# thobotics/geometry_rl

Measured on NVIDIA B200. Metric: fwd+bwd+TRPL update samples/sec (policy fwd+bwd, TRPL projection, losses, critic, Adam), higher is better.
Workload: dtype bf16

## Files before the change

### geometry_rl_b200/csrc/grl_conv_node_tc.cu

```cuda
#include <cuda.h>

#include "grl_common.cuh"
#include "grl_tc.cuh"

namespace grl {

constexpr int kLDX = 72;

constexpr int kNF2Threads = 512;
constexpr int kK1 = 80;

struct NodeFwd2Group {
  union {
    struct {
      float X1[kTM * kC];
      float X2[kTM * kLDX];
    } x;
    __half A1[kTM * kK1];
  } u;
};

struct NodeFwd2Smem {
  __half W1h[kH * kK1];
  __half W2h[kC * kH];
  NodeFwd2Group g[2];
  float b2[kC], bias[kC], lng[kC], lnb[kC];
  uint64_t bar[2][2];
  uint64_t bar_x[2];
  uint64_t bar_d[2];
  uint32_t tmem_base;
};

__device__ __forceinline__ void stage_x1_dense(float* __restrict__ X1, const float* __restrict__ src, int cnt, int gt,
                                               uint64_t* bar) {
  if (gt == 0) {
    tc::mbar_expect_tx(bar, (uint32_t)cnt * kRow * 4u);
    tc::bulk_g2s(X1, src, (uint32_t)cnt * kRow * 4u, bar);
  }
  if (cnt < kTE) {
#pragma unroll
    for (int i = 0; i < 8; ++i) {
      const int f = gt + 256 * i;
      if ((f >> 8) >= cnt) *reinterpret_cast<float4*>(X1 + 4 * f) = make_float4(0.f, 0.f, 0.f, 0.f);
    }
  }
}

template <bool kAcc>
__global__ void __launch_bounds__(kNF2Threads, 1) fbconv_node_fwd_tc2_kernel(const GrlConvDesc d, const __grid_constant__ CUtensorMap tm_xd) {
  extern __shared__ unsigned char smem_raw[];
  NodeFwd2Smem& s = *reinterpret_cast<NodeFwd2Smem*>(
      smem_raw + ((1024u - (tc::smem_u32(smem_raw) & 1023u)) & 1023u));
  const int tid = threadIdx.x;
  const int grp = tid >> 8, gt = tid & 255, gw = gt >> 5, lane = tid & 31;
  NodeFwd2Group& G = s.g[grp];
  const int bar_id = 1 + grp;

  if (tid == 0) {
    tc::mbar_init(&s.bar[0][0], 1);
    tc::mbar_init(&s.bar[0][1], 1);
    tc::mbar_init(&s.bar[1][0], 1);
    tc::mbar_init(&s.bar[1][1], 1);
    tc::mbar_init(&s.bar_x[0], 1);
    tc::mbar_init(&s.bar_x[1], 1);
    tc::mbar_init(&s.bar_d[0], 1);
    tc::mbar_init(&s.bar_d[1], 1);
    tc::fence_mbar_init();
  }
  if (tid < 32) tc::tmem_alloc(&s.tmem_base, 512);
  tc::stage_weight_f16(s.W1h, d.w1, kH, kC, kC);
  tc::stage_weight_f16(s.W2h, d.w2, kC, kH, kH);
  for (int n = tid; n < kH; n += kNF2Threads) {
    const float b = d.b1[n];
    const __half hi = __float2half_rn(b);
    const __half lo = __float2half_rn(b - __half2float(hi));
    const __half z = __float2half_rn(0.f);
    const __half2 h[4] = {__halves2half2(hi, lo), __halves2half2(z, z), __halves2half2(z, z), __halves2half2(z, z)};
    *reinterpret_cast<uint4*>(s.W1h + ((size_t)8 * kH + n) * 8) = tc::pack_h8(h);
    *reinterpret_cast<uint4*>(s.W1h + ((size_t)9 * kH + n) * 8) = make_uint4(0u, 0u, 0u, 0u);
  }
  if (tid < kC) { s.b2[tid] = d.b2[tid]; s.bias[tid] = d.bias[tid]; s.lng[tid] = d.ln_g[tid]; s.lnb[tid] = d.ln_b[tid]; }
  const int fc = gt & 63, pq = gt >> 6;
  unsigned long long fk2[kO][2];
#pragma unroll
  for (int o = 0; o < kO; ++o)
#pragma unroll
    for (int pi = 0; pi < 2; ++pi)
      fk2[o][pi] = pack2(__ldg(d.fiber_kernel + ((size_t)(o * kO + 4 * pq + 2 * pi)) * kC + fc) * 0.0625f,
                         __ldg(d.fiber_kernel + ((size_t)(o * kO + 4 * pq + 2 * pi + 1)) * kC + fc) * 0.0625f);

  const int n_tiles = (d.n_dst + kTE - 1) / kTE;
  const int tile_stride = 2 * gridDim.x;
  int tile = 2 * blockIdx.x + grp;
  tc::fence_async_smem();
  tc::tc_fence_before();
  __syncthreads();
  tc::tc_fence_after();
  if (tile < n_tiles)
    stage_x1_dense(G.u.x.X1, d.x1 + (size_t)tile * kTE * kRow, min(kTE, d.n_dst - tile * kTE), gt, &s.bar_x[grp]);
  const uint32_t tmem = s.tmem_base + 256u * grp;
  const uint32_t a1_addr = tc::smem_u32(G.u.A1);
  const uint32_t w1_addr = tc::smem_u32(s.W1h), w2_addr = tc::smem_u32(s.W2h);
  const int q = gw & 3, hh = gw >> 2;
  const int row = 32 * q + lane;
  const uint32_t lane_addr = tmem + ((uint32_t)(32 * q) << 16);
  uint32_t parity = 0;

  for (; tile < n_tiles; tile += tile_stride) {
    const int n0 = tile * kTE;
    if (gt == 0) {
      tc::prefetch_l2(d.x_dst + (size_t)n0 * kRow, (uint32_t)min(kTE, d.n_dst - n0) * kRow * 4u);
      const int nt = tile + tile_stride;
      if (nt < n_tiles) tc::prefetch_l2(d.x1 + (size_t)nt * kTE * kRow, (uint32_t)min(kTE, d.n_dst - nt * kTE) * kRow * 4u);
    }
    tc::mbar_wait(&s.bar_x[grp], parity);
    tc::group_sync(bar_id, 256);

    {
      const float bias_c = s.bias[fc];
#pragma unroll 2
      for (int j = 0; j < kTE; ++j) {
        unsigned long long a01 = pack2(0.f, 0.f), a23 = a01;
#pragma unroll
        for (int o = 0; o < kO; ++o) {
          const float x = G.u.x.X1[(16 * j + o) * kC + fc];
          const unsigned long long xx = pack2(x, x);
          a01 = ffma2(xx, fk2[o][0], a01);
          a23 = ffma2(xx, fk2[o][1], a23);
        }
        float a0, a1, a2, a3;
        unpack2(a01, a0, a1);
        unpack2(a23, a2, a3);
        float* o2 = G.u.x.X2 + (16 * j + 4 * pq) * kLDX + fc;
        o2[0 * kLDX] = a0 + bias_c;
        o2[1 * kLDX] = a1 + bias_c;
        o2[2 * kLDX] = a2 + bias_c;
        o2[3 * kLDX] = a3 + bias_c;
      }
    }
    tc::group_sync(bar_id, 256);

    {
      const int r = gt >> 1, h = gt & 1;
      float4 v[8];
      float sum = 0.f;
#pragma unroll
      for (int i = 0; i < 8; ++i) {
        v[i] = ld4(G.u.x.X2 + r * kLDX + 4 * (2 * i + h));
        sum += (v[i].x + v[i].y) + (v[i].z + v[i].w);
      }
      if (d.x2 && n0 + (r >> 4) < d.n_dst) {
        float* xo = d.x2 + (size_t)(n0 + (r >> 4)) * kRow + (r & 15) * kC + 4 * h;
#pragma unroll
        for (int i = 0; i < 8; ++i) st4(xo + 8 * i, v[i]);
      }
      sum += __shfl_xor_sync(0xffffffffu, sum, 1);
      const float mean = sum * (1.0f / 64.0f);
      float sq = 0.f;
#pragma unroll
      for (int i = 0; i < 8; ++i) {
        v[i].x -= mean; v[i].y -= mean; v[i].z -= mean; v[i].w -= mean;
        sq += (v[i].x * v[i].x + v[i].y * v[i].y) + (v[i].z * v[i].z + v[i].w * v[i].w);
      }
      sq += __shfl_xor_sync(0xffffffffu, sq, 1);
      const float rstd = rsqrtf(sq * (1.0f / 64.0f) + 1e-5f);
#pragma unroll
      for (int i = 0; i < 8; ++i) {
        const int c = 4 * (2 * i + h);
        const float4 g = ld4(s.lng + c), b = ld4(s.lnb + c);
        const __half2 p0 = __floats2half2_rn(v[i].x * rstd * g.x + b.x, v[i].y * rstd * g.y + b.y);
        const __half2 p1 = __floats2half2_rn(v[i].z * rstd * g.z + b.z, v[i].w * rstd * g.w + b.w);
        uint2 pk;
        pk.x = *reinterpret_cast<const uint32_t*>(&p0);
        pk.y = *reinterpret_cast<const uint32_t*>(&p1);
        *reinterpret_cast<uint2*>(G.u.A1 + ((size_t)i * kTM + r) * 8 + 4 * h) = pk;
      }
      *reinterpret_cast<uint4*>(G.u.A1 + ((size_t)(8 + h) * kTM + r) * 8) = make_uint4(h == 0 ? 0x3C003C00u : 0u, 0u, 0u, 0u);
    }
    tc::fence_async_smem();
    tc::tc_fence_before();
    tc::group_sync(bar_id, 256);
    if (gt == 0) {
      tc::tc_fence_after();
      tc::issue_mma_rolled(tmem, tc::view_k(a1_addr, kTM), tc::view_k(w1_addr, kH), tc::idesc_f16_ex(128, kH, 0, 0, 0, 0), kK1 / 16, false);
      tc::mma_commit(&s.bar[grp][0]);
      tc::mbar_expect_tx(&s.bar_d[grp], 2u * kTM * 32u * 4u);
      tc::tma_load_2d(G.u.x.X2, &tm_xd, 0, n0 * kO, &s.bar_d[grp]);
      tc::tma_load_2d(G.u.x.X2 + kTM * 32, &tm_xd, 32, n0 * kO, &s.bar_d[grp]);
    }
    tc::mbar_wait(&s.bar[grp][0], parity);
    tc::tc_fence_after();
    {
      const int nt = tile + tile_stride;
      if (nt < n_tiles) {
        tc::fence_async_smem();
        stage_x1_dense(G.u.x.X1, d.x1 + (size_t)nt * kTE * kRow, min(kTE, d.n_dst - nt * kTE), gt, &s.bar_x[grp]);
      }
    }
    {
#pragma unroll 2
      for (int i = 0; i < 8; ++i) {
        const int c0 = 128 * hh + 16 * i;
        float v[16];
        tc::tmem_ld16(lane_addr + c0, v);
        uint32_t r[8];
#pragma unroll
        for (int e = 0; e < 4; ++e) {
          const __half2 a = tc::gelu_h2(__floats2half2_rn(v[2 * e], v[2 * e + 1]));
          const __half2 b = tc::gelu_h2(__floats2half2_rn(v[8 + 2 * e], v[8 + 2 * e + 1]));
          r[e] = *reinterpret_cast<const uint32_t*>(&a);
          r[4 + e] = *reinterpret_cast<const uint32_t*>(&b);
        }
        tc::tmem_st8(lane_addr + 128 * hh + 8 * i, r);
      }
      tc::tmem_st_wait();
    }
    tc::tc_fence_before();
    tc::group_sync(bar_id, 256);
    if (gt == 0) {
      tc::tc_fence_after();
      const tc::OpView w2v = tc::view_k(w2_addr, kC);
      tc::OpView w2hi = w2v;
      w2hi.addr += 8 * w2v.adv;
      tc::issue_mma_ts(tmem + 64, tmem, w2v, tc::idesc_f16_ex(128, kC, 0, 0, 0, 0), 8, false);
      tc::issue_mma_ts(tmem + 64, tmem + 128, w2hi, tc::idesc_f16_ex(128, kC, 0, 0, 0, 0), 8, true);
      tc::mma_commit(&s.bar[grp][1]);
    }
    const int node = n0 + (row >> 4);
    const bool live = node < d.n_dst;
    const size_t off = (size_t)(live ? node : 0) * kRow + (row & 15) * kC + 32 * hh;
    tc::mbar_wait(&s.bar[grp][1], parity);
    tc::tc_fence_after();
    tc::mbar_wait(&s.bar_d[grp], parity);
    const float* xrow = G.u.x.X2 + hh * (kTM * 32) + row * 32;
#pragma unroll
    for (int i = 0; i < 2; ++i) {
      float v[16];
      tc::tmem_ld16(lane_addr + 64 + 32 * hh + 16 * i, v);
      if (live) {
#pragma unroll
        for (int e = 0; e < 4; ++e) {
          const float4 bb = ld4(s.b2 + 32 * hh + 16 * i + 4 * e);
          float4 x = ld4(xrow + (((4 * i + e) ^ (row & 7)) << 2));
          if (kAcc) {
            const float4 old = ldg4(d.out + off + 16 * i + 4 * e);
            x.x += old.x; x.y += old.y; x.z += old.z; x.w += old.w;
          }
          st4(d.out + off + 16 * i + 4 * e, make_float4(x.x + (v[4 * e] + bb.x), x.y + (v[4 * e + 1] + bb.y),
                                                       x.z + (v[4 * e + 2] + bb.z), x.w + (v[4 * e + 3] + bb.w)));
        }
      }
    }
    tc::tc_fence_before();
    parity ^= 1u;
  }
  cp_async_wait_all();
  tc::tc_fence_before();
  __syncthreads();
  if (tid < 32) tc::tmem_dealloc(s.tmem_base, 512);
}

}

extern "C" int grl_fbconv_node_fwd_tc(const GrlConvDesc* d, grl_stream_t stream) {
  GRL_REQUIRE(d && d->n_dst > 0, GRL_EINVAL, "grl_fbconv_node_fwd_tc: bad descriptor");
  GRL_REQUIRE(d->x1 && d->fiber_kernel && d->bias && d->ln_g && d->ln_b && d->w1 && d->b1 && d->w2 && d->b2 && d->x_dst &&
                  d->out, GRL_EINVAL, "grl_fbconv_node_fwd_tc: null pointer");
  const int n_tiles = (d->n_dst + grl::kTE - 1) / grl::kTE;
  const int smem2 = (int)sizeof(grl::NodeFwd2Smem) + 1024;
  if (grl::ensure_dynamic_smem((const void*)grl::fbconv_node_fwd_tc2_kernel<false>, smem2) != GRL_OK) return GRL_ECUDA;
  if (grl::ensure_dynamic_smem((const void*)grl::fbconv_node_fwd_tc2_kernel<true>, smem2) != GRL_OK) return GRL_ECUDA;
  alignas(64) CUtensorMap tm_xd;
  if (grl::make_row_tensor_map(&tm_xd, d->x_dst, d->n_dst, grl::kTM) != GRL_OK) return GRL_ECUDA;
  int grid = grl::sm_count();
  if (2 * grid > n_tiles) grid = (n_tiles + 1) / 2;
  if (d->accumulate_out) grl::fbconv_node_fwd_tc2_kernel<true><<<grid, grl::kNF2Threads, smem2, (cudaStream_t)stream>>>(*d, tm_xd);
  else grl::fbconv_node_fwd_tc2_kernel<false><<<grid, grl::kNF2Threads, smem2, (cudaStream_t)stream>>>(*d, tm_xd);
  return grl::check_launch("grl_fbconv_node_fwd_tc");
}
```

### geometry_rl_b200/csrc/grl_tc.cuh

```cuda
#pragma once
#include <cuda_bf16.h>
#include <cuda_fp16.h>
#include <cuda_runtime.h>
#include <stdint.h>

namespace grl {
namespace tc {

__device__ __forceinline__ uint32_t smem_u32(const void* p) { return static_cast<uint32_t>(__cvta_generic_to_shared(p)); }

__device__ __forceinline__ void mbar_init(uint64_t* bar, uint32_t count) {
  asm volatile("mbarrier.init.shared::cta.b64 [%0], %1;" ::"r"(smem_u32(bar)), "r"(count) : "memory");
}
__device__ __forceinline__ void fence_mbar_init() { asm volatile("fence.mbarrier_init.release.cluster;" ::: "memory"); }
__device__ __forceinline__ void mbar_wait(uint64_t* bar, uint32_t parity) {
  const uint32_t addr = smem_u32(bar);
  uint32_t done;
  do {
    asm volatile(
        "{\n\t"
        ".reg .pred p;\n\t"
        "mbarrier.try_wait.parity.shared::cta.b64 p, [%1], %2;\n\t"
        "selp.u32 %0, 1, 0, p;\n\t"
        "}"
        : "=r"(done)
        : "r"(addr), "r"(parity)
        : "memory");
  } while (!done);
}

__device__ __forceinline__ void mbar_expect_tx(uint64_t* bar, uint32_t bytes) {
  asm volatile("mbarrier.arrive.expect_tx.shared::cta.b64 _, [%0], %1;" ::"r"(smem_u32(bar)), "r"(bytes) : "memory");
}
__device__ __forceinline__ void bulk_g2s(void* smem_dst, const void* gsrc, uint32_t bytes, uint64_t* bar) {
  asm volatile("cp.async.bulk.shared::cluster.global.mbarrier::complete_tx::bytes [%0], [%1], %2, [%3];" ::"r"(
                   smem_u32(smem_dst)),
               "l"(gsrc), "r"(bytes), "r"(smem_u32(bar))
               : "memory");
}

__device__ __forceinline__ void tma_load_2d(void* smem_dst, const void* tmap, int c0, int c1, uint64_t* bar) {
  asm volatile("cp.async.bulk.tensor.2d.shared::cluster.global.mbarrier::complete_tx::bytes [%0], [%1, {%2, %3}], [%4];" ::"r"(
                   smem_u32(smem_dst)),
               "l"(tmap), "r"(c0), "r"(c1), "r"(smem_u32(bar))
               : "memory");
}
__device__ __forceinline__ void tma_prefetch_desc(const void* tmap) {
  asm volatile("prefetch.tensormap [%0];" ::"l"(tmap) : "memory");
}

__device__ __forceinline__ void fence_async_smem() { asm volatile("fence.proxy.async.shared::cta;" ::: "memory"); }
__device__ __forceinline__ void tc_fence_before() { asm volatile("tcgen05.fence::before_thread_sync;" ::: "memory"); }
__device__ __forceinline__ void tc_fence_after() { asm volatile("tcgen05.fence::after_thread_sync;" ::: "memory"); }

__device__ __forceinline__ void tmem_alloc(uint32_t* smem_dst, uint32_t ncols) {
  asm volatile("tcgen05.alloc.cta_group::1.sync.aligned.shared::cta.b32 [%0], %1;" ::"r"(smem_u32(smem_dst)), "r"(ncols)
               : "memory");
  asm volatile("tcgen05.relinquish_alloc_permit.cta_group::1.sync.aligned;" ::: "memory");
}
__device__ __forceinline__ void tmem_dealloc(uint32_t taddr, uint32_t ncols) {
  asm volatile("tcgen05.dealloc.cta_group::1.sync.aligned.b32 %0, %1;" ::"r"(taddr), "r"(ncols) : "memory");
}

__device__ __forceinline__ uint64_t smem_desc(uint32_t saddr, uint32_t lbo_bytes, uint32_t sbo_bytes) {
  uint64_t d = 0;
  d |= (uint64_t)((saddr >> 4) & 0x3FFF);
  d |= (uint64_t)((lbo_bytes >> 4) & 0x3FFF) << 16;
  d |= (uint64_t)((sbo_bytes >> 4) & 0x3FFF) << 32;
  d |= (uint64_t)1 << 46;
  return d;
}
__host__ __device__ constexpr uint32_t idesc_bf16(int M, int N) {
  return (1u << 4) | (1u << 7) | (1u << 10) | ((uint32_t)(N >> 3) << 17) | ((uint32_t)(M >> 4) << 24);
}

__host__ __device__ constexpr uint32_t idesc_f16_ex(int M, int N, int a_mn, int b_mn, int a_bf16, int b_bf16) {
  return (1u << 4) | ((uint32_t)a_bf16 << 7) | ((uint32_t)b_bf16 << 10) | ((uint32_t)a_mn << 15) | ((uint32_t)b_mn << 16) |
         ((uint32_t)(N >> 3) << 17) | ((uint32_t)(M >> 4) << 24);
}

__device__ __forceinline__ void mma_bf16(uint32_t tmem_d, uint64_t desc_a, uint64_t desc_b, uint32_t idesc, uint32_t accumulate) {
  asm volatile(
      "{\n\t"
      ".reg .pred p;\n\t"
      "setp.ne.b32 p, %4, 0;\n\t"
      "tcgen05.mma.cta_group::1.kind::f16 [%0], %1, %2, %3, p;\n\t"
      "}" ::"r"(tmem_d),
      "l"(desc_a), "l"(desc_b), "r"(idesc), "r"(accumulate)
      : "memory");
}
__device__ __forceinline__ void mma_commit(uint64_t* bar) {
  asm volatile("tcgen05.commit.cta_group::1.mbarrier::arrive::one.shared::cluster.b64 [%0];" ::"r"(smem_u32(bar)) : "memory");
}

template <int N, int K>
__device__ __forceinline__ void issue_gemm(uint32_t tmem_d, uint32_t a_saddr, int a_rows, uint32_t b_saddr, int b_rows,
                                           bool accumulate_first) {
  constexpr uint32_t idesc = idesc_bf16(128, N);
#pragma unroll
  for (int k = 0; k < K / 16; ++k) {
    const uint64_t da = smem_desc(a_saddr + k * 2 * a_rows * 16, a_rows * 16, 128);
    const uint64_t db = smem_desc(b_saddr + k * 2 * b_rows * 16, b_rows * 16, 128);
    mma_bf16(tmem_d, da, db, idesc, (k > 0 || accumulate_first) ? 1u : 0u);
  }
}

struct OpView {
  uint32_t addr, lbo, sbo, adv;
};
__device__ __forceinline__ OpView view_k(uint32_t addr, int rows) { return OpView{addr, (uint32_t)rows * 16u, 128u, (uint32_t)rows * 32u}; }
__device__ __forceinline__ OpView view_mn(uint32_t addr, int rows) { return OpView{addr, 128u, (uint32_t)rows * 16u, 256u}; }
__host__ __device__ constexpr uint32_t idesc_bf16_ex(int M, int N, int a_mn, int b_mn) {
  return idesc_bf16(M, N) | ((uint32_t)a_mn << 15) | ((uint32_t)b_mn << 16);
}
struct Op {
  uint32_t lo, hi, step;
};
__device__ __forceinline__ uint32_t desc_lo(uint32_t saddr, uint32_t lbo_bytes) {
  return ((saddr >> 4) & 0x3FFFu) | (((lbo_bytes >> 4) & 0x3FFFu) << 16);
}
__device__ __forceinline__ uint32_t desc_hi(uint32_t sbo_bytes) { return ((sbo_bytes >> 4) & 0x3FFFu) | (1u << 14); }
__device__ __forceinline__ Op op_k(uint32_t addr, int rows) { return Op{desc_lo(addr, (uint32_t)rows * 16u), desc_hi(128u), (uint32_t)rows * 2u}; }
__device__ __forceinline__ Op op_mn(uint32_t addr, int rows) { return Op{desc_lo(addr, 128u), desc_hi((uint32_t)rows * 16u), 16u}; }
__device__ __forceinline__ void mma_f16_words(uint32_t tmem_d, uint32_t alo, uint32_t ahi, uint32_t blo, uint32_t bhi, uint32_t idesc,
                                              uint32_t accumulate) {
  asm volatile(
      "{\n\t"
      ".reg .pred p;\n\t"
      ".reg .b64 da, db;\n\t"
      "setp.ne.b32 p, %6, 0;\n\t"
      "mov.b64 da, {%1, %2};\n\t"
      "mov.b64 db, {%3, %4};\n\t"
      "tcgen05.mma.cta_group::1.kind::f16 [%0], da, db, %5, p;\n\t"
      "}" ::"r"(tmem_d),
      "r"(alo), "r"(ahi), "r"(blo), "r"(bhi), "r"(idesc), "r"(accumulate)
      : "memory");
}
template <int KSTEPS>
__device__ __forceinline__ void issue_mma_fast(uint32_t tmem_d, const Op& a, const Op& b, uint32_t idesc, bool accumulate_first) {
  mma_f16_words(tmem_d, a.lo, a.hi, b.lo, b.hi, idesc, accumulate_first ? 1u : 0u);
#pragma unroll
  for (int k = 1; k < KSTEPS; ++k) mma_f16_words(tmem_d, a.lo + k * a.step, a.hi, b.lo + k * b.step, b.hi, idesc, 1u);
}
__device__ __forceinline__ void mma_f16_ts(uint32_t tmem_d, uint32_t tmem_a, uint32_t blo, uint32_t bhi, uint32_t idesc,
                                           uint32_t accumulate) {
  asm volatile(
      "{\n\t"
      ".reg .pred p;\n\t"
      ".reg .b64 db;\n\t"
      "setp.ne.b32 p, %5, 0;\n\t"
      "mov.b64 db, {%2, %3};\n\t"
      "tcgen05.mma.cta_group::1.kind::f16 [%0], [%1], db, %4, p;\n\t"
      "}" ::"r"(tmem_d),
      "r"(tmem_a), "r"(blo), "r"(bhi), "r"(idesc), "r"(accumulate)
      : "memory");
}
__device__ __forceinline__ void issue_mma_ts(uint32_t tmem_d, uint32_t tmem_a, const OpView& b, uint32_t idesc, int ksteps,
                                             bool accumulate_first) {
  const uint32_t blo = desc_lo(b.addr, b.lbo), bhi = desc_hi(b.sbo), bs = b.adv >> 4;
#pragma unroll
  for (int k = 0; k < ksteps; ++k)
    mma_f16_ts(tmem_d, tmem_a + 8u * k, blo + k * bs, bhi, idesc, (k > 0 || accumulate_first) ? 1u : 0u);
}

__device__ __forceinline__ void issue_mma(uint32_t tmem_d, const OpView& a, const OpView& b, uint32_t idesc, int ksteps,
                                          bool accumulate_first) {
  const uint32_t alo = desc_lo(a.addr, a.lbo), ahi = desc_hi(a.sbo), blo = desc_lo(b.addr, b.lbo), bhi = desc_hi(b.sbo);
  const uint32_t as = a.adv >> 4, bs = b.adv >> 4;
#pragma unroll
  for (int k = 0; k < ksteps; ++k)
    mma_f16_words(tmem_d, alo + k * as, ahi, blo + k * bs, bhi, idesc, (k > 0 || accumulate_first) ? 1u : 0u);
}
__device__ __forceinline__ void issue_mma_rolled(uint32_t tmem_d, const OpView& a, const OpView& b, uint32_t idesc, int ksteps,
                                                 bool accumulate_first) {
  uint32_t alo = desc_lo(a.addr, a.lbo), blo = desc_lo(b.addr, b.lbo);
  const uint32_t ahi = desc_hi(a.sbo), bhi = desc_hi(b.sbo), as = a.adv >> 4, bs = b.adv >> 4;
  mma_f16_words(tmem_d, alo, ahi, blo, bhi, idesc, accumulate_first ? 1u : 0u);
#pragma unroll 1
  for (int k = 1; k < ksteps; ++k) {
    alo += as;
    blo += bs;
    mma_f16_words(tmem_d, alo, ahi, blo, bhi, idesc, 1u);
  }
}
__device__ __forceinline__ bool elect_one() {
  uint32_t pred;
  asm volatile(
      "{\n\t"
      ".reg .pred p;\n\t"
      "elect.sync _|p, 0xffffffff;\n\t"
      "selp.u32 %0, 1, 0, p;\n\t"
      "}"
      : "=r"(pred));
  return pred != 0;
}

template <int NV>
__device__ __forceinline__ void warp_colsum(float (&v)[NV], int lane) {
  static_assert(NV % 32 == 0, "NV must be a multiple of 32");
#pragma unroll
  for (int step = 0; step < 5; ++step) {
    const int half = NV >> (step + 1);
    const int bit = 16 >> step;
    const bool upper = (lane & bit) != 0;
#pragma unroll
    for (int i = 0; i < half; ++i) {
      const float keep = upper ? v[i + half] : v[i];
      const float send = upper ? v[i] : v[i + half];
      v[i] = keep + __shfl_xor_sync(0xffffffffu, send, bit);
    }
  }
}

__device__ __forceinline__ void tmem_ld16(uint32_t taddr, float (&v)[16]) {
  uint32_t r[16];
  asm volatile(
      "tcgen05.ld.sync.aligned.32x32b.x16.b32 {%0, %1, %2, %3, %4, %5, %6, %7, %8, %9, %10, %11, %12, %13, %14, %15}, [%16];"
      : "=r"(r[0]), "=r"(r[1]), "=r"(r[2]), "=r"(r[3]), "=r"(r[4]), "=r"(r[5]), "=r"(r[6]), "=r"(r[7]), "=r"(r[8]),
        "=r"(r[9]), "=r"(r[10]), "=r"(r[11]), "=r"(r[12]), "=r"(r[13]), "=r"(r[14]), "=r"(r[15])
      : "r"(taddr)
      : "memory");
  asm volatile("tcgen05.wait::ld.sync.aligned;" ::: "memory");
#pragma unroll
  for (int i = 0; i < 16; ++i) v[i] = __uint_as_float(r[i]);
}

__device__ __forceinline__ void tmem_st16(uint32_t taddr, const uint32_t (&r)[16]) {
  asm volatile(
      "tcgen05.st.sync.aligned.32x32b.x16.b32 [%0], {%1, %2, %3, %4, %5, %6, %7, %8, %9, %10, %11, %12, %13, %14, %15, %16};" ::"r"(taddr),
      "r"(r[0]), "r"(r[1]), "r"(r[2]), "r"(r[3]), "r"(r[4]), "r"(r[5]), "r"(r[6]), "r"(r[7]), "r"(r[8]), "r"(r[9]), "r"(r[10]),
      "r"(r[11]), "r"(r[12]), "r"(r[13]), "r"(r[14]), "r"(r[15])
      : "memory");
}
__device__ __forceinline__ void tmem_st8(uint32_t taddr, const uint32_t (&r)[8]) {
  asm volatile("tcgen05.st.sync.aligned.32x32b.x8.b32 [%0], {%1, %2, %3, %4, %5, %6, %7, %8};" ::"r"(taddr), "r"(r[0]), "r"(r[1]),
               "r"(r[2]), "r"(r[3]), "r"(r[4]), "r"(r[5]), "r"(r[6]), "r"(r[7])
               : "memory");
}
__device__ __forceinline__ void tmem_st_wait() { asm volatile("tcgen05.wait::st.sync.aligned;" ::: "memory"); }
__device__ __forceinline__ void tmem_ld16_raw(uint32_t taddr, uint32_t (&r)[16]) {
  asm volatile(
      "tcgen05.ld.sync.aligned.32x32b.x16.b32 {%0, %1, %2, %3, %4, %5, %6, %7, %8, %9, %10, %11, %12, %13, %14, %15}, [%16];"
      : "=r"(r[0]), "=r"(r[1]), "=r"(r[2]), "=r"(r[3]), "=r"(r[4]), "=r"(r[5]), "=r"(r[6]), "=r"(r[7]), "=r"(r[8]),
        "=r"(r[9]), "=r"(r[10]), "=r"(r[11]), "=r"(r[12]), "=r"(r[13]), "=r"(r[14]), "=r"(r[15])
      : "r"(taddr)
      : "memory");
  asm volatile("tcgen05.wait::ld.sync.aligned;" ::: "memory");
}
__device__ __forceinline__ void mbar_arrive(uint64_t* bar) {
  asm volatile("mbarrier.arrive.shared::cta.b64 _, [%0];" ::"r"(smem_u32(bar)) : "memory");
}

__device__ __forceinline__ void prefetch_l2(const void* gptr, uint32_t bytes) {
  asm volatile("cp.async.bulk.prefetch.L2.global [%0], %1;" ::"l"(gptr), "r"(bytes) : "memory");
}

__device__ __forceinline__ void group_sync(int id, int count) { asm volatile("bar.sync %0, %1;" ::"r"(id), "r"(count) : "memory"); }

__device__ __forceinline__ __half2 tanh_h2(__half2 x) {
  uint32_t r;
  asm("tanh.approx.f16x2 %0, %1;" : "=r"(r) : "r"(*reinterpret_cast<uint32_t*>(&x)));
  return *reinterpret_cast<__half2*>(&r);
}
__device__ __forceinline__ __half2 gelu_h2(__half2 x) {
  const __half2 k = __floats2half2_rn(0.7978845608028654f, 0.7978845608028654f);
  const __half2 kc = __floats2half2_rn(0.7978845608028654f * 0.044715f, 0.7978845608028654f * 0.044715f);
  const __half2 half = __floats2half2_rn(0.5f, 0.5f);
  const __half2 t = tanh_h2(__hmul2(x, __hfma2(__hmul2(x, x), kc, k)));
  const __half2 hx = __hmul2(x, half);
  return __hfma2(hx, t, hx);
}
__device__ __forceinline__ void gelu_h2(__half2 x, __half2& y, __half2& dy) {
  const __half2 k = __floats2half2_rn(0.7978845608028654f, 0.7978845608028654f);
  const __half2 kc = __floats2half2_rn(0.7978845608028654f * 0.044715f, 0.7978845608028654f * 0.044715f);
  const __half2 kh = __floats2half2_rn(0.5f * 0.7978845608028654f, 0.5f * 0.7978845608028654f);
  const __half2 k3h = __floats2half2_rn(1.5f * 0.7978845608028654f * 0.044715f, 1.5f * 0.7978845608028654f * 0.044715f);
  const __half2 half = __floats2half2_rn(0.5f, 0.5f), one = __floats2half2_rn(1.0f, 1.0f);
  const __half2 x2max = __floats2half2_rn(1024.0f, 1024.0f);
  const __half2 x2 = __hmul2(x, x);
  const __half2 t = tanh_h2(__hmul2(x, __hfma2(x2, kc, k)));
  const __half2 e = __hfma2(t, half, half);
  y = __hmul2(x, e);
  dy = __hfma2(__hmul2(x, __hfma2(__hneg2(t), t, one)), __hfma2(__hmin2(x2, x2max), k3h, kh), e);
}
__device__ __forceinline__ uint4 pack_h8(const __half2 (&h)[4]) {
  uint4 o;
  o.x = *reinterpret_cast<const uint32_t*>(&h[0]);
  o.y = *reinterpret_cast<const uint32_t*>(&h[1]);
  o.z = *reinterpret_cast<const uint32_t*>(&h[2]);
  o.w = *reinterpret_cast<const uint32_t*>(&h[3]);
  return o;
}

__device__ __forceinline__ int op_index(int rows, int row, int k) { return ((k >> 3) * rows + row) * 8 + (k & 7); }

__device__ __forceinline__ uint4 pack8(const float* v) {
  __nv_bfloat162 a = __floats2bfloat162_rn(v[0], v[1]);
  __nv_bfloat162 b = __floats2bfloat162_rn(v[2], v[3]);
  __nv_bfloat162 c = __floats2bfloat162_rn(v[4], v[5]);
  __nv_bfloat162 d = __floats2bfloat162_rn(v[6], v[7]);
  uint4 o;
  o.x = *reinterpret_cast<uint32_t*>(&a);
  o.y = *reinterpret_cast<uint32_t*>(&b);
  o.z = *reinterpret_cast<uint32_t*>(&c);
  o.w = *reinterpret_cast<uint32_t*>(&d);
  return o;
}

__device__ __forceinline__ uint4 pack8_h(const float* v) {
  const __half2 a = __floats2half2_rn(v[0], v[1]), b = __floats2half2_rn(v[2], v[3]);
  const __half2 c = __floats2half2_rn(v[4], v[5]), d = __floats2half2_rn(v[6], v[7]);
  uint4 o;
  o.x = *reinterpret_cast<const uint32_t*>(&a);
  o.y = *reinterpret_cast<const uint32_t*>(&b);
  o.z = *reinterpret_cast<const uint32_t*>(&c);
  o.w = *reinterpret_cast<const uint32_t*>(&d);
  return o;
}

__device__ __forceinline__ float grad_scale_from_amax(uint32_t amax_bits) {
  const int e = (int)((amax_bits >> 23) & 0xFFu);
  if (e == 0 || e == 255) return 1.0f;
  int k = 127 + 5 - (e - 127);
  k = k < 1 ? 1 : (k > 254 ? 254 : k);
  return __uint_as_float((uint32_t)k << 23);
}

__device__ __forceinline__ void stage_weight_bf16(__nv_bfloat16* dst, const float* __restrict__ src, int rows, int K, int ld) {
  const int n_chunks = rows * (K >> 3);
  for (int i = threadIdx.x; i < n_chunks; i += blockDim.x) {
    const int row = i % rows, kc = i / rows;
    const float4 lo = __ldg(reinterpret_cast<const float4*>(src + (size_t)row * ld + kc * 8));
    const float4 hi = __ldg(reinterpret_cast<const float4*>(src + (size_t)row * ld + kc * 8 + 4));
    const float v[8] = {lo.x, lo.y, lo.z, lo.w, hi.x, hi.y, hi.z, hi.w};
    *reinterpret_cast<uint4*>(dst + ((size_t)kc * rows + row) * 8) = pack8(v);
  }
}

__device__ __forceinline__ void stage_weight_f16(__half* dst, const float* __restrict__ src, int rows, int K, int ld) {
  const int n_chunks = rows * (K >> 3);
  for (int i = threadIdx.x; i < n_chunks; i += blockDim.x) {
    const int row = i % rows, kc = i / rows;
    const float4 lo = __ldg(reinterpret_cast<const float4*>(src + (size_t)row * ld + kc * 8));
    const float4 hi = __ldg(reinterpret_cast<const float4*>(src + (size_t)row * ld + kc * 8 + 4));
    const __half2 h[4] = {__floats2half2_rn(lo.x, lo.y), __floats2half2_rn(lo.z, lo.w), __floats2half2_rn(hi.x, hi.y),
                          __floats2half2_rn(hi.z, hi.w)};
    *reinterpret_cast<uint4*>(dst + ((size_t)kc * rows + row) * 8) = pack_h8(h);
  }
}

}
}
```

Baseline: 971,900.

## Write node-conv x2 and output tiles via swizzled smem and TMA stores

Moves X2 out of the union into its own 1024-byte-aligned swizzled buffer. The x2 intermediate and the final output are now written to global memory by asynchronous TMA bulk tensor stores instead of per-thread vector stores. The epilogue writes its results back into smem and one thread issues the stores, with bulk wait_group.read guarding buffer reuse. This is meant to make global writes asynchronous and coalesced, at the cost of more shared memory per group, extra group barriers, and a different LayerNorm row mapping.

```diff
diff --git a/geometry_rl_b200/csrc/grl_conv_node_tc.cu b/geometry_rl_b200/csrc/grl_conv_node_tc.cu
--- a/geometry_rl_b200/csrc/grl_conv_node_tc.cu
+++ b/geometry_rl_b200/csrc/grl_conv_node_tc.cu
@@ -5,19 +5,15 @@
 
 namespace grl {
 
-constexpr int kLDX = 72;
-
 constexpr int kNF2Threads = 512;
 constexpr int kK1 = 80;
 
 struct NodeFwd2Group {
   union {
-    struct {
-      float X1[kTM * kC];
-      float X2[kTM * kLDX];
-    } x;
+    float X1[kTM * kC];
     __half A1[kTM * kK1];
   } u;
+  float X2[kTM * kC];
 };
 
 struct NodeFwd2Smem {
@@ -30,6 +26,12 @@
   uint64_t bar_d[2];
   uint32_t tmem_base;
 };
+static_assert(offsetof(NodeFwd2Smem, g) % 1024 == 0 && sizeof(NodeFwd2Group) % 1024 == 0 &&
+                  offsetof(NodeFwd2Group, X2) % 1024 == 0, "X2 must be 1024-byte aligned");
+
+__device__ __forceinline__ int swz(int row, int c) {
+  return (c >> 5) * (kTM * 32) + row * 32 + ((((c & 31) >> 2) ^ (row & 7)) << 2) + (c & 3);
+}
 
 __device__ __forceinline__ void stage_x1_dense(float* __restrict__ X1, const float* __restrict__ src, int cnt, int gt,
                                                uint64_t* bar) {
@@ -47,7 +49,9 @@
 }
 
 template <bool kAcc>
-__global__ void __launch_bounds__(kNF2Threads, 1) fbconv_node_fwd_tc2_kernel(const GrlConvDesc d, const __grid_constant__ CUtensorMap tm_xd) {
+__global__ void __launch_bounds__(kNF2Threads, 1)
+    fbconv_node_fwd_tc2_kernel(const GrlConvDesc d, const __grid_constant__ CUtensorMap tm_xd,
+                               const __grid_constant__ CUtensorMap tm_x2, const __grid_constant__ CUtensorMap tm_out) {
   extern __shared__ unsigned char smem_raw[];
   NodeFwd2Smem& s = *reinterpret_cast<NodeFwd2Smem*>(
       smem_raw + ((1024u - (tc::smem_u32(smem_raw) & 1023u)) & 1023u));
@@ -97,13 +101,15 @@
   __syncthreads();
   tc::tc_fence_after();
   if (tile < n_tiles)
-    stage_x1_dense(G.u.x.X1, d.x1 + (size_t)tile * kTE * kRow, min(kTE, d.n_dst - tile * kTE), gt, &s.bar_x[grp]);
+    stage_x1_dense(G.u.X1, d.x1 + (size_t)tile * kTE * kRow, min(kTE, d.n_dst - tile * kTE), gt, &s.bar_x[grp]);
   const uint32_t tmem = s.tmem_base + 256u * grp;
   const uint32_t a1_addr = tc::smem_u32(G.u.A1);
   const uint32_t w1_addr = tc::smem_u32(s.W1h), w2_addr = tc::smem_u32(s.W2h);
   const int q = gw & 3, hh = gw >> 2;
   const int row = 32 * q + lane;
   const uint32_t lane_addr = tmem + ((uint32_t)(32 * q) << 16);
+  const int ln_h = lane & 1;
+  const int ln_r = 16 * gw + 8 * (lane >> 4) + 2 * ((lane >> 1) & 3) + ((lane >> 3) & 1);
   uint32_t parity = 0;
 
   for (; tile < n_tiles; tile += tile_stride) {
@@ -112,6 +118,7 @@
       tc::prefetch_l2(d.x_dst + (size_t)n0 * kRow, (uint32_t)min(kTE, d.n_dst - n0) * kRow * 4u);
       const int nt = tile + tile_stride;
       if (nt < n_tiles) tc::prefetch_l2(d.x1 + (size_t)nt * kTE * kRow, (uint32_t)min(kTE, d.n_dst - nt * kTE) * kRow * 4u);
+      tc::bulk_wait_read_all();
     }
     tc::mbar_wait(&s.bar_x[grp], parity);
     tc::group_sync(bar_id, 256);
@@ -123,7 +130,7 @@
         unsigned long long a01 = pack2(0.f, 0.f), a23 = a01;
 #pragma unroll
         for (int o = 0; o < kO; ++o) {
-          const float x = G.u.x.X1[(16 * j + o) * kC + fc];
+          const float x = G.u.X1[(16 * j + o) * kC + fc];
           const unsigned long long xx = pack2(x, x);
           a01 = ffma2(xx, fk2[o][0], a01);
           a23 = ffma2(xx, fk2[o][1], a23);
@@ -131,28 +138,29 @@
         float a0, a1, a2, a3;
         unpack2(a01, a0, a1);
         unpack2(a23, a2, a3);
-        float* o2 = G.u.x.X2 + (16 * j + 4 * pq) * kLDX + fc;
-        o2[0 * kLDX] = a0 + bias_c;
-        o2[1 * kLDX] = a1 + bias_c;
-        o2[2 * kLDX] = a2 + bias_c;
-        o2[3 * kLDX] = a3 + bias_c;
-      }
-    }
-    tc::group_sync(bar_id, 256);
+        const int r0 = 16 * j + 4 * pq;
+        G.X2[swz(r0 + 0, fc)] = a0 + bias_c;
+        G.X2[swz(r0 + 1, fc)] = a1 + bias_c;
+        G.X2[swz(r0 + 2, fc)] = a2 + bias_c;
+        G.X2[swz(r0 + 3, fc)] = a3 + bias_c;
+      }
+    }
+    tc::fence_async_smem();
+    tc::group_sync(bar_id, 256);
+    if (gt == 0 && d.x2) {
+      tc::tma_store_2d(&tm_x2, G.X2, 0, n0 * kO);
+      tc::tma_store_2d(&tm_x2, G.X2 + kTM * 32, 32, n0 * kO);
+      tc::bulk_commit();
+    }
 
     {
-      const int r = gt >> 1, h = gt & 1;
+      const int r = ln_r, h = ln_h;
       float4 v[8];
       float sum = 0.f;
 #pragma unroll
       for (int i = 0; i < 8; ++i) {
-        v[i] = ld4(G.u.x.X2 + r * kLDX + 4 * (2 * i + h));
+        v[i] = ld4(G.X2 + swz(r, 4 * (2 * i + h)));
         sum += (v[i].x + v[i].y) + (v[i].z + v[i].w);
-      }
-      if (d.x2 && n0 + (r >> 4) < d.n_dst) {
-        float* xo = d.x2 + (size_t)(n0 + (r >> 4)) * kRow + (r & 15) * kC + 4 * h;
-#pragma unroll
-        for (int i = 0; i < 8; ++i) st4(xo + 8 * i, v[i]);
       }
       sum += __shfl_xor_sync(0xffffffffu, sum, 1);
       const float mean = sum * (1.0f / 64.0f);
@@ -184,9 +192,10 @@
       tc::tc_fence_after();
       tc::issue_mma_rolled(tmem, tc::view_k(a1_addr, kTM), tc::view_k(w1_addr, kH), tc::idesc_f16_ex(128, kH, 0, 0, 0, 0), kK1 / 16, false);
       tc::mma_commit(&s.bar[grp][0]);
+      tc::bulk_wait_read_all();
       tc::mbar_expect_tx(&s.bar_d[grp], 2u * kTM * 32u * 4u);
-      tc::tma_load_2d(G.u.x.X2, &tm_xd, 0, n0 * kO, &s.bar_d[grp]);
-      tc::tma_load_2d(G.u.x.X2 + kTM * 32, &tm_xd, 32, n0 * kO, &s.bar_d[grp]);
+      tc::tma_load_2d(G.X2, &tm_xd, 0, n0 * kO, &s.bar_d[grp]);
+      tc::tma_load_2d(G.X2 + kTM * 32, &tm_xd, 32, n0 * kO, &s.bar_d[grp]);
     }
     tc::mbar_wait(&s.bar[grp][0], parity);
     tc::tc_fence_after();
@@ -194,7 +203,7 @@
       const int nt = tile + tile_stride;
       if (nt < n_tiles) {
         tc::fence_async_smem();
-        stage_x1_dense(G.u.x.X1, d.x1 + (size_t)nt * kTE * kRow, min(kTE, d.n_dst - nt * kTE), gt, &s.bar_x[grp]);
+        stage_x1_dense(G.u.X1, d.x1 + (size_t)nt * kTE * kRow, min(kTE, d.n_dst - nt * kTE), gt, &s.bar_x[grp]);
       }
     }
     {
@@ -232,7 +241,7 @@
     tc::mbar_wait(&s.bar[grp][1], parity);
     tc::tc_fence_after();
     tc::mbar_wait(&s.bar_d[grp], parity);
-    const float* xrow = G.u.x.X2 + hh * (kTM * 32) + row * 32;
+    float* xrow = G.X2 + hh * (kTM * 32) + row * 32;
 #pragma unroll
     for (int i = 0; i < 2; ++i) {
       float v[16];
@@ -241,20 +250,29 @@
 #pragma unroll
         for (int e = 0; e < 4; ++e) {
           const float4 bb = ld4(s.b2 + 32 * hh + 16 * i + 4 * e);
-          float4 x = ld4(xrow + (((4 * i + e) ^ (row & 7)) << 2));
+          float* xp = xrow + (((4 * i + e) ^ (row & 7)) << 2);
+          float4 x = ld4(xp);
           if (kAcc) {
             const float4 old = ldg4(d.out + off + 16 * i + 4 * e);
             x.x += old.x; x.y += old.y; x.z += old.z; x.w += old.w;
           }
-          st4(d.out + off + 16 * i + 4 * e, make_float4(x.x + (v[4 * e] + bb.x), x.y + (v[4 * e + 1] + bb.y),
-                                                       x.z + (v[4 * e + 2] + bb.z), x.w + (v[4 * e + 3] + bb.w)));
+          const float4 o = make_float4(x.x + (v[4 * e] + bb.x), x.y + (v[4 * e + 1] + bb.y), x.z + (v[4 * e + 2] + bb.z),
+                                       x.w + (v[4 * e + 3] + bb.w));
+          st4(xp, o);
         }
       }
     }
     tc::tc_fence_before();
+    tc::fence_async_smem();
+    tc::group_sync(bar_id, 256);
+    if (gt == 0) {
+      tc::tma_store_2d(&tm_out, G.X2, 0, n0 * kO);
+      tc::tma_store_2d(&tm_out, G.X2 + kTM * 32, 32, n0 * kO);
+      tc::bulk_commit();
+    }
     parity ^= 1u;
   }
-  cp_async_wait_all();
+  if (gt == 0) tc::bulk_wait_all();
   tc::tc_fence_before();
   __syncthreads();
   if (tid < 32) tc::tmem_dealloc(s.tmem_base, 512);
@@ -270,11 +288,14 @@
   const int smem2 = (int)sizeof(grl::NodeFwd2Smem) + 1024;
   if (grl::ensure_dynamic_smem((const void*)grl::fbconv_node_fwd_tc2_kernel<false>, smem2) != GRL_OK) return GRL_ECUDA;
   if (grl::ensure_dynamic_smem((const void*)grl::fbconv_node_fwd_tc2_kernel<true>, smem2) != GRL_OK) return GRL_ECUDA;
-  alignas(64) CUtensorMap tm_xd;
+  alignas(64) CUtensorMap tm_xd, tm_x2, tm_out;
   if (grl::make_row_tensor_map(&tm_xd, d->x_dst, d->n_dst, grl::kTM) != GRL_OK) return GRL_ECUDA;
+  if (d->x2 && grl::make_row_tensor_map(&tm_x2, d->x2, d->n_dst, grl::kTM) != GRL_OK) return GRL_ECUDA;
+  if (!d->x2) tm_x2 = tm_xd;
+  if (grl::make_row_tensor_map(&tm_out, d->out, d->n_dst, grl::kTM) != GRL_OK) return GRL_ECUDA;
   int grid = grl::sm_count();
   if (2 * grid > n_tiles) grid = (n_tiles + 1) / 2;
-  if (d->accumulate_out) grl::fbconv_node_fwd_tc2_kernel<true><<<grid, grl::kNF2Threads, smem2, (cudaStream_t)stream>>>(*d, tm_xd);
-  else grl::fbconv_node_fwd_tc2_kernel<false><<<grid, grl::kNF2Threads, smem2, (cudaStream_t)stream>>>(*d, tm_xd);
+  if (d->accumulate_out) grl::fbconv_node_fwd_tc2_kernel<true><<<grid, grl::kNF2Threads, smem2, (cudaStream_t)stream>>>(*d, tm_xd, tm_x2, tm_out);
+  else grl::fbconv_node_fwd_tc2_kernel<false><<<grid, grl::kNF2Threads, smem2, (cudaStream_t)stream>>>(*d, tm_xd, tm_x2, tm_out);
   return grl::check_launch("grl_fbconv_node_fwd_tc");
 }
diff --git a/geometry_rl_b200/csrc/grl_tc.cuh b/geometry_rl_b200/csrc/grl_tc.cuh
--- a/geometry_rl_b200/csrc/grl_tc.cuh
+++ b/geometry_rl_b200/csrc/grl_tc.cuh
@@ -45,6 +45,14 @@
                "l"(tmap), "r"(c0), "r"(c1), "r"(smem_u32(bar))
                : "memory");
 }
+__device__ __forceinline__ void tma_store_2d(const void* tmap, const void* smem_src, int c0, int c1) {
+  asm volatile("cp.async.bulk.tensor.2d.global.shared::cta.bulk_group [%0, {%1, %2}], [%3];" ::"l"(tmap), "r"(c0), "r"(c1),
+               "r"(smem_u32(smem_src))
+               : "memory");
+}
+__device__ __forceinline__ void bulk_commit() { asm volatile("cp.async.bulk.commit_group;" ::: "memory"); }
+__device__ __forceinline__ void bulk_wait_read_all() { asm volatile("cp.async.bulk.wait_group.read 0;" ::: "memory"); }
+__device__ __forceinline__ void bulk_wait_all() { asm volatile("cp.async.bulk.wait_group 0;" ::: "memory"); }
 __device__ __forceinline__ void tma_prefetch_desc(const void* tmap) {
   asm volatile("prefetch.tensormap [%0];" ::"l"(tmap) : "memory");
 }
```

Result: faster. 1.021 million, median of 6 (+5.0%).
